# HKU-BAL/MegaPath-Nano

Hardware: AMD Instinct MI355X
Metric: Gbp/min ONT reads aligned+species-assigned vs RefSeq, 1/2/4/8 MI355X (higher is better)
Workload: dtype int32

## Files before the change

megapath_nano_amd/csrc/align.hip:

```cpp
#include "map_types.h"
#include "ext_kernels.h"
#include "fin_kernels.h"
#include "tag_kernels.h"
#include "stitch_kernels.h"
#include "plan_kernels.h"
#include "hit_kernels.h"
#include "mapper_internal.h"
#include "../../include/mpn_map.h"
#include "../../include/mpn_ssw.h"

#include <algorithm>
#include <condition_variable>
#include <deque>
#include <math.h>
#include <stdio.h>
#include <string.h>
#include <thread>
#include <pthread.h>
#include <time.h>
#include <atomic>
#include <functional>
#include <mutex>
#include <stdlib.h>
#include <string>
// ... 764 lines not shown
    int n_jobs = 0;
};

struct HostSeqs { const char *seqs; const int64_t *seq_off; const int32_t *seq_len; const int64_t *tseq_off; };

static int run_job_group(const RefView &rv, const mpn_map_opt *opt, int nj_cap, const unsigned long long *d_nj, DevRound &dv, const uint8_t *d_reads,
                         const int64_t *d_read_off, const int32_t *d_read_len, int64_t budget, const HostSeqs *hs, StreamLease &st) {
    if (nj_cap == 0) return 0;
    int nj = nj_cap;
    WallTimer wt;
    Slot &SL = *tl_slot;
    const int strip_scores = ext_strip_scores_ok(opt->a, -opt->b, -opt->sc_ambi, opt->q + opt->e, opt->q2 + opt->e2) ? 1 : 0;
    ExtParams prm;
    prm.sc_mch = (int8_t)opt->a; prm.sc_mis = (int8_t)-opt->b; prm.sc_n = (int8_t)-opt->sc_ambi;
    prm.q = (int8_t)opt->q; prm.e = (int8_t)opt->e; prm.q2 = (int8_t)opt->q2; prm.e2 = (int8_t)opt->e2; prm.zdrop_thres = opt->zdrop;
    prm.zdrop_inv = opt->zdrop_inv; prm.max_gap = opt->max_gap;
    const size_t order_cap = (size_t)nj + (size_t)N_STRIP * 8 + 16;
    if (SL.pool_sizes.ensure((size_t)nj * sizeof(JobSizes) + 16) || SL.pool_buckets.ensure((size_t)2 * N_BUCKETS * 4 + sizeof(LayoutTotals) + 16) ||
        SL.pool_order.ensure(order_cap * 4) || SL.pin_res.ensure(sizeof(LayoutTotals) + 96) ||
        SL.pool_redo_ids.ensure((size_t)nj * 4 + 16) || SL.pool_probes.ensure((size_t)nj * sizeof(InvProbe) + 16))
        return -1;
    struct { ExtJob *p; } d_jobs{dv.jobs};
    JobSizes *d_sizes = SL.pool_sizes.as<JobSizes>();
    int32_t *d_bcnt = SL.pool_buckets.as<int32_t>(), *d_bcur = d_bcnt + N_BUCKETS;
    LayoutTotals *d_tot = reinterpret_cast<LayoutTotals *>(d_bcnt + 2 * N_BUCKETS);
    struct { int32_t *p; } d_order{SL.pool_order.as<int32_t>()};
    {
        ZeroList z{};
        zero_list_push(z, d_bcnt, (size_t)2 * N_BUCKETS * 4 + sizeof(LayoutTotals));
        zero_list_push(z, dv.used + 1, 8);
        zero_list_push(z, dv.used + 5, 8);
        zero_list_push(z, dv.used + 8, 16);
        zero_list_push(z, dv.used + 7, 8);
        MPN_HIP_CHECK(zero_regions(z, st));
    }
    const int lay_grid = std::max(1, std::min((nj + 255) / 256, 256));
    EvTimer evl(st);
    static const bool tiled_on = []() { const char *e = getenv("MPN_TILED"); return !e || atoi(e) != 0; }();
    static const int tile_pick = []() { const char *e = getenv("MPN_TILE_CLASS"); return e ? std::min(std::max(atoi(e), 0), N_TILE_CLASS - 1) : -1; }();
    hipLaunchKernelGGL(job_classify_kernel, dim3(lay_grid), dim3(256), 0, st, d_jobs.p, d_nj, strip_scores, prm, g_force_kernel ? g_force_kernel : (tiled_on ? 0 : 7),
                       tile_pick, d_sizes, d_bcnt, d_tot);
    hipLaunchKernelGGL(job_scan_kernel, dim3(1), dim3(1024), 0, st, d_sizes, d_nj, (const int32_t *)d_bcnt, d_bcur, d_tot, d_order.p);
    hipLaunchKernelGGL(job_layout_kernel, dim3(lay_grid), dim3(256), 0, st, d_jobs.p, d_nj, (const JobSizes *)d_sizes, d_bcur, d_order.p);
    MPN_HIP_CHECK(hipGetLastError());
    LayoutTotals *h_tot = SL.pin_res.as<LayoutTotals>();
    evl.mark(56);
    MPN_HIP_CHECK(hipMemcpyAsync(h_tot, d_tot, sizeof(LayoutTotals), hipMemcpyDeviceToHost, st));
    MPN_HIP_CHECK(stream_sync(st));
    evl.resolve();
    const LayoutTotals T = *h_tot;
    nj = T.n_jobs;
    dv.n_jobs = nj;
    if (nj == 0) return 0;
    if (T.too_large) { set_error("DP window too large for LDS staging (%d x %d)", T.tl_q, T.tl_t); return -4; }
    if (!dv.compact) {
        if (SL.pool_compact.ensure((size_t)T.cig_tot * 4 * 2 + 16)) return -1;
        dv.compact = SL.pool_compact.as<uint32_t>();
        dv.cig_cap = T.cig_tot;
    }
    if (budget > 0 && T.p_tot > budget && nj > 1) return 1;
    const int *cnt = T.cnt, *base = T.base;
    g_stats[4] += nj; g_stats[5] += T.cells; g_stats[31] += T.strip_cells[0] + T.strip_cells[1] + T.strip_cells[2];
    for (int c = 0; c < 3; ++c) g_stats[41 + c] += T.strip_cells[c];
    g_stats[58] += T.xstrip_cells;
    for (int c = 0; c < N_TILE_CLASS; ++c) {
        g_stats[64] += cnt[L_TILE + c];
        g_stats[STAT_TILE_CLASS + c] += cnt[L_TILE + c];
    }
    if (getenv("MPN_DEBUG_JOBS")) {
        static const char *const fam[] = {"wg64", "wg", "strip", "band", "tile"};
        for (int l = 0; l < N_LISTS; ++l)
            if (cnt[l]) fprintf(stderr, "[jobs] %s list %-2d n=%d\n", fam[l < L_WG ? 0 : l < L_STRIP ? 1 : l < L_BAND ? 2 : l < L_TILE ? 3 : 4], l, cnt[l]);
    }
    if (const char *dump = getenv("MPN_DUMP_STRIPS")) {
        const int n_ord = base[L_BAND] - base[L_STRIP];
        std::vector<int32_t> ord(n_ord);
        std::vector<ExtJob> hj(nj);
        MPN_HIP_CHECK(hipMemcpy(ord.data(), d_order.p + base[L_STRIP], (size_t)n_ord * 4, hipMemcpyDeviceToHost));
        MPN_HIP_CHECK(hipMemcpy(hj.data(), d_jobs.p, (size_t)nj * sizeof(ExtJob), hipMemcpyDeviceToHost));
        static std::mutex mu;
        std::lock_guard<std::mutex> lk(mu);
        if (const char *all = getenv("MPN_DUMP_JOBS"))
            if (FILE *f = fopen(all, "ab")) {
                for (int j = 0; j < nj; ++j) {
                    const int32_t rec[6] = {hj[j].cls, hj[j].qlen, hj[j].tlen, hj[j].w, hj[j].flag, hj[j].n_col};
                    fwrite(rec, 4, 6, f);
                }
                fclose(f);
            }
        if (FILE *f = fopen(dump, "ab")) {
            for (int l = L_STRIP; l < L_BAND; ++l)
                for (int k = base[l]; k < base[l + 1]; ++k) {
                    const int jid = ord[k - base[L_STRIP]];
                    const int32_t rec[4] = {strip_glc_of_list(l), jid >= 0 ? hj[jid].qlen : 0, jid >= 0 ? hj[jid].tlen : 0, jid >= 0 ? hj[jid].strip_s : 0};
                    fwrite(rec, 4, 4, f);
                }
            fclose(f);
        }
    }
    if (SL.pool_P.ensure((size_t)T.p_tot + 16) || SL.pool_OFF.ensure((size_t)T.row_tot * 2 * 4 + 16) ||
        SL.pool_state.ensure((size_t)T.state_tot + 16) || SL.pool_CIG.ensure((size_t)T.cig_tot * 4 + 16))
        return -1;
    wt.stop_into(g_stats[27]);
    struct { uint8_t *p; } P{SL.pool_P.as<uint8_t>()};
    struct { int32_t *p; } OFF{SL.pool_OFF.as<int32_t>()};
    struct { int8_t *p; } gstate{SL.pool_state.as<int8_t>()};
    struct { uint32_t *p; } CIG{SL.pool_CIG.as<uint32_t>()};
    struct { ExtRes *p; } d_res{dv.res};
    uint32_t *d_compact = dv.compact;
    unsigned long long *d_used = dv.used;
    int32_t *d_redo_ids = SL.pool_redo_ids.as<int32_t>();
    InvProbe *d_probes = SL.pool_probes.as<InvProbe>();
    auto launch_list = [&](int l, const int32_t *ord, int n, hipStream_t s) -> int {
        if (n == 0) return 0;
        if (l < L_STRIP) {
            const int ntc = (l - L_LDS) / 5;
            const size_t lds = std::max<size_t>((size_t)T.lds_need[(l - L_LDS) % 5], 64);
#define MPN_WG_LAUNCH(NT)                                                                                                             \
            do {                                                                                                                      \
                if (lds > 64 * 1024) MPN_HIP_CHECK(hipFuncSetAttribute((const void *)ext_dp_wg_kernel<NT>, hipFuncAttributeMaxDynamicSharedMemorySize, (int)lds)); \
                hipLaunchKernelGGL(ext_dp_wg_kernel<NT>, dim3(n), dim3(NT), lds, s, d_jobs.p, ord, n, prm, d_reads, d_read_off, d_read_len, \
                                   rv, P.p, OFF.p, gstate.p, d_res.p);                                                                \
            } while (0)
            if (ntc == 0) MPN_WG_LAUNCH(64); else if (ntc == 1) MPN_WG_LAUNCH(256); else if (ntc == 2) MPN_WG_LAUNCH(512); else MPN_WG_LAUNCH(1024);
#undef MPN_WG_LAUNCH
        } else if (l < L_BAND) {
            const int fam = (l - L_STRIP) / 48;
            StripSegs segs;
            segs.n = 0;
            int blocks = 0;
            size_t lds = 0;
            const int c_lo = fam == 0 ? 0 : 3, c_hi = fam == 0 ? 3 : N_STRIP_CLASS;
            for (int glc = 2; glc >= 0; --glc)
                for (int sclass = c_lo + glc; sclass < c_hi; sclass += 3) {
                    const int l0 = L_STRIP + 16 * sclass, nl = base[l0 + 16] - base[l0], per = strip_windows_per_wave(l0);
                    if (nl == 0) continue;
                    const int stride = (std::max(T.strip_lds[sclass], 16) + 3) & ~3;
                    const int nr_stride = fam ? T.strip_nr[sclass] + 16 : 0;
                    lds = std::max(lds, (size_t)stride * per + STRIP_TAB_BYTES + (size_t)per * 8 * nr_stride);
                    segs.s[segs.n++] = StripSeg{blocks, nl, base[l0], stride, nr_stride, glc, sclass >= 6 ? 1 : 0};
                    blocks += nl / per;
                }
            if (blocks == 0) return 0;
#define MPN_STRIP_LAUNCH(EX)                                                                                                          \
            do {                                                                                                                      \
                if (lds > 64 * 1024) MPN_HIP_CHECK(hipFuncSetAttribute((const void *)ext_dp_strip_kernel<EX>, hipFuncAttributeMaxDynamicSharedMemorySize, (int)lds)); \
                hipLaunchKernelGGL(ext_dp_strip_kernel<EX>, dim3(blocks), dim3(64), lds, s, d_jobs.p, (const int32_t *)d_order.p, segs, prm, d_reads, \
                                   d_read_off, d_read_len, rv, P.p, d_res.p);                                                         \
            } while (0)
            if (fam == 0) MPN_STRIP_LAUNCH(false); else MPN_STRIP_LAUNCH(true);
#undef MPN_STRIP_LAUNCH
        } else if (l >= L_TILE) {
            const int c = l - L_TILE;
            const size_t lds = (size_t)std::max(T.tile_lds[c], 64);
#define MPN_TILE_LAUNCH(S, NW)                                                                                                        \
            do {                                                                                                                      \
                if (lds > 64 * 1024) MPN_HIP_CHECK(hipFuncSetAttribute((const void *)ext_dp_tile_kernel<S, NW>, hipFuncAttributeMaxDynamicSharedMemorySize, (int)lds)); \
                hipLaunchKernelGGL((ext_dp_tile_kernel<S, NW>), dim3(n), dim3(64 * NW), lds, s, d_jobs.p, ord, n, prm, d_reads, d_read_off, \
                                   d_read_len, rv, P.p, gstate.p, d_res.p, d_used + 7);                                              \
            } while (0)
            static_assert(N_TILE_CLASS == 4, "tile classes");
            if (c == 0) MPN_TILE_LAUNCH(16, 1); else if (c == 1) MPN_TILE_LAUNCH(4, 8); else if (c == 2) MPN_TILE_LAUNCH(8, 4); else MPN_TILE_LAUNCH(4, 16);
#undef MPN_TILE_LAUNCH
        } else {
            const int bvar = (l - L_BAND) / 4;
            const size_t lds = std::max<size_t>((size_t)T.band_lds[(l - L_BAND) % 4], 64);
// ... 2080 lines not shown
```

megapath_nano_amd/csrc/ext_kernels.h:

```cpp
#pragma once
#include "mpn_common.h"
#include "map_types.h"

namespace mpn {

enum { EZ_APPROX_MAX = 0x02, EZ_RIGHT = 0x08, EZ_EXTZ_ONLY = 0x40, EZ_REV_CIGAR = 0x80 };

struct ExtJob {
    int32_t read;
    int32_t rid;
    int32_t rev;
    int32_t qs, qlen;
    int32_t ts, tlen;
    int32_t reversed;
    int32_t w, zdrop, end_bonus, flag;
    int64_t p_off;
    int64_t row_off;
    int64_t cig_off;
    int32_t n_col;
    int32_t state_mode;
    int64_t state_off;
    int32_t layout;
    int32_t qstride;
    int32_t strip_s;
// ... 852 lines not shown
                                                         const int n_list, const ExtParams &prm, const uint8_t *__restrict__ reads,
                                                         const int64_t *__restrict__ read_off, const int32_t *__restrict__ read_len,
                                                         const RefView &rv, uint8_t *__restrict__ P, ExtRes *__restrict__ res, uint8_t *smem,
                                                         const int lds_stride, const int nr_stride) {
    const int j0 = first < n_list ? order[first] : -1;
    if (j0 < 0) return;
    const int S = jobs[j0].strip_s;
#define MPN_CASE(SS) case SS: ext_strip_exact<SS, GL, RIGHT>(jobs, order, first, n_list, prm, reads, read_off, read_len, rv, P, res, smem, lds_stride, nr_stride); break
    switch (S) {
        MPN_CASE(1); MPN_CASE(2); MPN_CASE(3); MPN_CASE(4); MPN_CASE(5); MPN_CASE(6); MPN_CASE(7); MPN_CASE(8);
        MPN_CASE(9); MPN_CASE(10); MPN_CASE(11); MPN_CASE(12); MPN_CASE(13); MPN_CASE(14); MPN_CASE(15);
        default: ext_strip_exact<16, GL, RIGHT>(jobs, order, first, n_list, prm, reads, read_off, read_len, rv, P, res, smem, lds_stride, nr_stride); break;
    }
#undef MPN_CASE
}

struct StripSeg { int32_t first_block, n_list, ord_off, lds_stride, nr_stride, glc, right; };
struct StripSegs { StripSeg s[6]; int32_t n; };

template <bool EXACT>
__global__ __launch_bounds__(64) __attribute__((amdgpu_waves_per_eu(3, 3))) void ext_dp_strip_kernel(const ExtJob *__restrict__ jobs, const int32_t *__restrict__ order, StripSegs segs,
                                                          ExtParams prm, const uint8_t *__restrict__ reads,
                                                          const int64_t *__restrict__ read_off, const int32_t *__restrict__ read_len,
                                                          RefView rv, uint8_t *__restrict__ P, ExtRes *__restrict__ res) {
    extern __shared__ __attribute__((aligned(16))) uint8_t smem[];
    int k = 0;
    while (k + 1 < segs.n && (int)blockIdx.x >= segs.s[k + 1].first_block) ++k;
    const StripSeg sg = segs.s[k];
    const int32_t *ord = order + sg.ord_off;
    if constexpr (!EXACT) {
        {
            const int first2 = ((int)blockIdx.x - sg.first_block) * (8 >> sg.glc);
            int S = 16;
            for (int k = 0; k < (8 >> sg.glc); ++k) { const int slot = first2 + k; if (slot < sg.n_list && ord[slot] >= 0) { S = jobs[ord[slot]].strip_s; break; } }
#define MPN_PAIR(SS, GLN) ext_strip_pair<SS, GLN>(jobs, ord, first2, sg.n_list, prm, reads, read_off, read_len, rv, P, res, smem, sg.lds_stride)
#define MPN_PAIR_S(GLN) switch (S) { case 1: MPN_PAIR(1, GLN); break; case 2: MPN_PAIR(2, GLN); break; case 3: MPN_PAIR(3, GLN); break; case 4: MPN_PAIR(4, GLN); break; \
            case 5: MPN_PAIR(5, GLN); break; case 6: MPN_PAIR(6, GLN); break; case 7: MPN_PAIR(7, GLN); break; case 8: MPN_PAIR(8, GLN); break; \
            case 9: MPN_PAIR(9, GLN); break; case 10: MPN_PAIR(10, GLN); break; case 11: MPN_PAIR(11, GLN); break; case 12: MPN_PAIR(12, GLN); break; \
            case 13: MPN_PAIR(13, GLN); break; case 14: MPN_PAIR(14, GLN); break; case 15: MPN_PAIR(15, GLN); break; default: MPN_PAIR(16, GLN); break; }
            if (sg.glc == 0) MPN_PAIR_S(16) else if (sg.glc == 1) MPN_PAIR_S(32) else MPN_PAIR_S(64)
#undef MPN_PAIR_S
#undef MPN_PAIR
        }
    } else {
        const int first = ((int)blockIdx.x - sg.first_block) * (4 >> sg.glc);
#define MPN_GL(GLN, RT) ext_strip_exact_dispatch<GLN, RT>(jobs, ord, first, sg.n_list, prm, reads, read_off, read_len, rv, P, res, smem, sg.lds_stride, sg.nr_stride)
        if (sg.right) { if (sg.glc == 0) MPN_GL(16, true); else if (sg.glc == 1) MPN_GL(32, true); else MPN_GL(64, true); }
        else { if (sg.glc == 0) MPN_GL(16, false); else if (sg.glc == 1) MPN_GL(32, false); else MPN_GL(64, false); }
#undef MPN_GL
    }
}

struct TileGeom { int T0, rows, n_lanes, W, jlo, jhi; int64_t base; };
__host__ __device__ inline TileGeom tile_geom(int tile, int qlen, int tlen, int w, int S) {
    const int R = 64 * S;
    TileGeom g{};
    g.T0 = tile * R;
    g.rows = tlen - g.T0 < R ? tlen - g.T0 : R;
    g.n_lanes = (g.rows + S - 1) / S;
    g.W = g.n_lanes * S;
    g.jlo = g.T0 - w > 0 ? g.T0 - w : 0;
    g.jhi = g.T0 + g.rows - 1 + w < qlen - 1 ? g.T0 + g.rows - 1 + w : qlen - 1;
    const int64_t m = tile;
    const int64_t k0 = (int64_t)w / R + 1;
    const int64_t n0 = m > k0 ? m - k0 : 0;
    const int64_t s_lo = (int64_t)R * (n0 * (k0 + m - 1) / 2) - n0 * (int64_t)w;
    const int64_t num = (int64_t)qlen - R - w;
    int64_t k1 = num <= 0 ? 0 : (num + R - 1) / R;
    if (k1 > m) k1 = m;
    const int64_t s_hi = (int64_t)R * (k1 * (k1 - 1) / 2) + k1 * (int64_t)(R - 1 + w) + (m - k1) * (int64_t)(qlen - 1);
    g.base = (s_hi - s_lo + 64 * m) * R;
    return g;
}
__host__ __device__ inline int64_t tile_matrix_bytes(int qlen, int tlen, int w, int S) {
    const int R = 64 * S, nt_all = (tlen + R - 1) / R, nt_band = (int)(((int64_t)qlen - 1 + w) / R) + 1, nt = nt_all < nt_band ? nt_all : nt_band;
    const TileGeom g = tile_geom(nt - 1, qlen, tlen, w, S);
    return g.base + (int64_t)((g.jhi >= g.jlo ? g.jhi - g.jlo + 1 : 0) + g.n_lanes - 1) * g.W;
}
__host__ __device__ inline bool ext_tile_ok(int qlen, int tlen, int w) {
    const int d = qlen > tlen ? qlen - tlen : tlen - qlen;
    return qlen > 0 && tlen > 0 && w >= 1 && d <= w && tlen <= 32768 && qlen <= 60000;
}

__host__ __device__ inline bool ext_tile_exact_ok(int mch, int mis, int amb, int q, int e, int q2, int e2, int qlen, int tlen, int w) {
    if (!(qlen > 0 && tlen > 0 && w >= 1 && tlen <= 8191 && qlen <= 16384 && qlen + tlen - 1 <= 14000)) return false;
    const int mn = qlen < tlen ? qlen : tlen, mx = qlen > tlen ? qlen : tlen;
    int worst = mis < amb ? -mis : -amb;
    if (worst < 0) worst = 0;
    const int g1 = worst * mn + q + e * (mx - mn + 1), g1b = q + e * (mx + 1), g2 = worst * mn + q2 + e2 * (mx - mn + 1), g2b = q2 + e2 * (mx + 1);
    const int lo1 = g1 > g1b ? g1 : g1b, lo2 = g2 > g2b ? g2 : g2b;
    return mch * mn < 32000 && (lo1 < lo2 ? lo1 : lo2) < 32000;
}
constexpr int TILE_RING_COLS = 2048, TILE_CTRL_BYTES = 4 * (2 * 16 + 4);
__host__ __device__ inline int ext_tile_ring_off(int qlen) { return ((qlen + 3) & ~3) + 64 + TILE_CTRL_BYTES; }
__host__ __device__ inline int ext_tile_lds_bytes(int qlen, int tlen, bool exact, int NW) {
    return ext_tile_ring_off(qlen) + (NW > 1 ? 12 * TILE_RING_COLS : 0) + (exact ? 8 * ((qlen + tlen + 2) & ~3) : 0);
}
__host__ __device__ inline bool ext_tile_pipe_ok(int w, int S, int NW) {
    return 2 * w + 128 < NW * (TILE_RING_COLS / NW + 64 * S);
}
constexpr int TILE_SPIN_MAX = 1 << 21;

template <int S, int NW, bool EXACT, bool RIGHT>
__device__ __forceinline__ void ext_tile_body(const ExtJob &jb, const int jid, const ExtParams &prm, const uint8_t *__restrict__ reads,
                                              const int64_t *__restrict__ read_off, const int32_t *__restrict__ read_len, const RefView &rv,
                                              uint8_t *__restrict__ P, int8_t *__restrict__ gstate, ExtRes *__restrict__ res, uint8_t *smem,
                                              unsigned long long *__restrict__ n_failed) {
    static_assert(S % 4 == 0 && S <= 16 && NW >= 1 && NW <= 16, "rows per lane: 4, 8, 12 or 16");
    constexpr int R = 64 * S, NT = 64 * NW;
    const int tid = threadIdx.x, lane = tid & 63, wave = tid >> 6;
    const int qlen = jb.qlen, tlen = jb.tlen;
    int q = prm.q, e = prm.e, q2 = prm.q2, e2 = prm.e2;
    if (q2 + e2 < q + e) { int t_ = q; q = q2; q2 = t_; t_ = e; e = e2; e2 = t_; }
    const int qe = q + e, qe2 = q2 + e2;
    int w = jb.w;
    if (w < 0) w = tlen > qlen ? tlen : qlen;
    ExtRes out;
    out.max = 0; out.zdropped = 0; out.max_q = out.max_t = out.mqe_t = -1; out.mqe = NEG_INF; out.score = NEG_INF;
    out.reach_end = 0; out.n_cigar = 0; out.r_done = -1; out.bt_i = out.bt_j = -1; out.do_bt = 0; out.zcode = 0; out.cig_pos = 0;
    if (!(EXACT ? ext_tile_exact_ok(prm.sc_mch, prm.sc_mis, prm.sc_n, prm.q, prm.e, prm.q2, prm.e2, qlen, tlen, w) : ext_tile_ok(qlen, tlen, w)) || -prm.sc_mis > 2 * (q + e) ||
        (NW > 1 && !ext_tile_pipe_ok(w, S, NW))) { if (tid == 0) res[jid] = out; return; }
    constexpr int RS = RIGHT ? 0 : 4, RA = RIGHT ? 1 : 3, RB = 2, RA2 = RIGHT ? 3 : 1, RB2 = RIGHT ? 4 : 0;
    const uint32_t sb_mch = (uint32_t)(8 * prm.sc_mch + RS + 128) & 0xff, sb_mis = (uint32_t)(8 * prm.sc_mis + RS + 128) & 0xff,
                   sb_n = (uint32_t)(8 * prm.sc_n + RS + 128) & 0xff;
    const int q_pad = (qlen + 3) & ~3;
    uint32_t *tab = reinterpret_cast<uint32_t *>(smem + q_pad);
    if (tid < 5) tab[tid] = lane == 4 ? sb_n * 0x01010101u : (sb_mis * 0x01010101u) ^ ((sb_mch ^ sb_mis) << (8 * lane));
    {
        const int64_t roff = read_off[jb.read];
        const int32_t rlen = read_len[jb.read];
        for (int i = tid; i < qlen; i += NT) smem[i] = (uint8_t)(4 * ext_qbase(reads, roff, rlen, jb.rev, jb.qs + (jb.reversed ? qlen - 1 - i : i)));
    }
    int long_thres = e != e2 ? (q2 - q) / (e - e2) - 1 : 0;
    if (q2 + e2 + long_thres * e2 > q + e + long_thres * e) ++long_thres;
    const int long_diff = long_thres * (e - e2) - (q2 - q) - e2;
#define MPN_BND(R) (8 * ((R) == 0 ? -qe : (R) < long_thres ? -e : (R) == long_thres ? long_diff : -e2))
    typedef short s16x2 __attribute__((ext_vector_type(2)));
    typedef unsigned short u16x2 __attribute__((ext_vector_type(2)));
    auto pk = [](int lo, int hi) { return (uint32_t)(hi * 65536 + lo); };
    constexpr int BETA = 0x2000 + 128;
    const int cv_lo = -8 * qe + RA + BETA, cv_hi = -8 * qe2 + RA2 + BETA, cu_lo = -8 * qe + RB + BETA, cu_hi = -8 * qe2 + RB2 + BETA;
    const uint32_t CV = pk(cv_lo, cv_hi), CU = pk(cu_lo, cu_hi);
    const uint32_t FRESH_U = pk(-8 * qe, -8 * qe) + CU, EDGE_V = pk(-8 * qe, -8 * qe) + CV;
    const uint32_t KONST = sb_n | 0x2000u;
    const uint32_t KZZ = pk(-16 * qe + RA + RB + BETA, -16 * qe2 + RA2 + RB2 + BETA);
    constexpr int RU = RIGHT ? 8 : 0;
    const uint32_t KEA = pk(8 * e - 8 * qe + RA - RU, 8 * e2 - 8 * qe2 + RA2 - RU), KEB = pk(8 * e - 8 * qe + RB - RU, 8 * e2 - 8 * qe2 + RB2 - RU);
    const uint32_t EIGHT = 0x00080008u, RANK_CLR = 0xfff8fff8u;
    const uint32_t MCH7 = (uint32_t)(8 * prm.sc_mch + 7 + BETA) * 0x00010001u;
    const int64_t g0 = rv.seq_off[jb.rid] + jb.ts;
    uint32_t *bnd_base = reinterpret_cast<uint32_t *>(gstate + jb.state_off);
    const int n_tiles = (tlen + R - 1) / R;
    uint32_t *ctrl = reinterpret_cast<uint32_t *>(smem + ext_tile_ring_off(qlen) - TILE_CTRL_BYTES);
    uint32_t *ring = ctrl + TILE_CTRL_BYTES / 4;
    constexpr int C = TILE_RING_COLS / NW;
    const int n_r = qlen + tlen - 1;
    uint32_t *BEST = reinterpret_cast<uint32_t *>(smem + ext_tile_ring_off(qlen) + (NW > 1 ? 12 * TILE_RING_COLS : 0)), *SE = BEST + ((n_r + 3) & ~3);
    int32_t *HL = reinterpret_cast<int32_t *>(NW > 1 ? bnd_base : bnd_base + 6 * (size_t)qlen);
    if (tid < 2 * NW + 1) ctrl[tid] = 0;
    if constexpr (EXACT) {
        for (int r = tid; r < n_r; r += NT) {
            int st = 0, en = tlen - 1;
            if (st < r - qlen + 1) st = r - qlen + 1;
            if (en > r) en = r;
            if (st < (r - w + 1) >> 1) st = (r - w + 1) >> 1;
            if (en > (r + w) >> 1) en = (r + w) >> 1;
            if (st > en) { st = 1; en = 0; }
            BEST[r] = 0;
            SE[r] = (uint32_t)st | (uint32_t)en << 16;
        }
        for (int t = tid; t < tlen; t += NT) HL[t] = NEG_INF;
        __builtin_amdgcn_fence(__ATOMIC_RELEASE, "agent");
    }
    __syncthreads();
    const bool head = lane == 0;
    int32_t score8 = 0;
    uint32_t *const prod_in = &ctrl[(wave + NW - 1) % NW], *const cons_in = &ctrl[NW + (wave + NW - 1) % NW];
    uint32_t *const prod_out = &ctrl[wave], *const cons_out = &ctrl[NW + wave];
    uint32_t *const ring_in = ring + 3 * C * ((wave + NW - 1) % NW), *const ring_out = ring + 3 * C * wave;
    uint32_t n_in = 0, n_out = 0, seen_prod = 0, seen_cons = 0;
    bool failed = false;
    auto wait_gt = [&](uint32_t *ctr, uint32_t lim, uint32_t &seen) -> bool {
        if ((int)(seen - lim) > 0) return true;
        for (int k = 0; k < TILE_SPIN_MAX; ++k) {
            seen = __hip_atomic_load(ctr, __ATOMIC_RELAXED, __HIP_MEMORY_SCOPE_WORKGROUP);
            if ((int)(seen - lim) > 0) return true;
            if (__hip_atomic_load(&ctrl[2 * NW], __ATOMIC_RELAXED, __HIP_MEMORY_SCOPE_WORKGROUP)) return false;
            __builtin_amdgcn_s_sleep(1);
        }
        __hip_atomic_store(&ctrl[2 * NW], 1u, __ATOMIC_RELAXED, __HIP_MEMORY_SCOPE_WORKGROUP);
        return false;
    };
    for (int tile = NW > 1 ? wave : 0; tile < n_tiles; tile += NW) {
        const TileGeom G = tile_geom(tile, qlen, tlen, w, S);
        const int T0 = G.T0, n_lanes = G.n_lanes, W = G.W, jlo = G.jlo, jhi = G.jhi;
        if (jhi < jlo) break;
        const int prev_jhi = tile > 0 ? min(qlen - 1, T0 - 1 + w) : -1;
        const int jlo_next = T0 + R - w > 0 ? T0 + R - w : 0;
        uint32_t *bnd_in = bnd_base + (size_t)(tile & 1) * 3 * (size_t)qlen, *bnd_out = bnd_base + (size_t)((tile + 1) & 1) * 3 * (size_t)qlen;
        const bool write_bnd = tile + 1 < n_tiles;
        const int t0 = T0 + lane * S;
        uint32_t UL[S], YL[S], TSEL[S];
        int32_t H8[S];
#pragma unroll
        for (int k = 0; k < S; ++k) {
            const int t = t0 + k;
            const int sq = t < tlen ? ref_code(rv, g0 + (jb.reversed ? tlen - 1 - t : t)) : 4;
            TSEL[k] = 0x0c0c0100u | (sq < 4 ? 4u + (uint32_t)sq : 0u);
            UL[k] = jlo == 0 ? pk(MPN_BND(t), MPN_BND(t)) + CU : FRESH_U;
            YL[k] = 0;
            H8[k] = 8 * (t < long_thres ? -(q + e * (t + 1)) : -(q2 + e2 * (t + 1)));
        }
        uint8_t *prow = P + jb.p_off + G.base + (int64_t)lane * S;
        const int n_steps = (jhi - jlo + 1) + n_lanes - 1;
        int out_v = 0, out_x = 0, out_h = 0;
        uint32_t qt = 0;
        auto qcode = [&](int col) -> uint32_t { return col < qlen ? (uint32_t)smem[col] : 16u; };
        uint32_t qt_next = *reinterpret_cast<const uint32_t *>(reinterpret_cast<const uint8_t *>(tab) + qcode(jlo));
        uint32_t qc_next = qcode(jlo + 1);
        uint32_t bv_n = 0, bx_n = 0, bh_n = 0, bv_n2 = 0, bx_n2 = 0, bh_n2 = 0;
        auto load_bnd = [&](int col, uint32_t &a, uint32_t &b, uint32_t &c) {
            if (tile > 0 && head && col <= prev_jhi && col < qlen) {
                if constexpr (NW == 1) { a = bnd_in[3 * (size_t)col]; b = bnd_in[3 * (size_t)col + 1]; c = bnd_in[3 * (size_t)col + 2]; }
                else {
                    const uint32_t n = n_in + (uint32_t)(col - jlo), slot = n % C;
                    if (!failed && !wait_gt(prod_in, n, seen_prod)) failed = true;
                    __atomic_signal_fence(__ATOMIC_SEQ_CST);
                    a = ring_in[slot]; b = ring_in[C + slot]; c = ring_in[2 * C + slot];
                    __atomic_signal_fence(__ATOMIC_SEQ_CST);
                    __hip_atomic_store(cons_in, n + 1, __ATOMIC_RELAXED, __HIP_MEMORY_SCOPE_WORKGROUP);
                }
            }
        };
        load_bnd(jlo, bv_n, bx_n, bh_n);
        load_bnd(jlo + 1, bv_n2, bx_n2, bh_n2);
        for (int step = 0; step < n_steps; ++step) {
            const uint32_t q_in = qt_next;
            qt_next = *reinterpret_cast<const uint32_t *>(reinterpret_cast<const uint8_t *>(tab) + qc_next);
            qc_next = qcode(jlo + step + 2);
            const uint32_t bv = bv_n, bx = bx_n, bh = bh_n;
            bv_n = bv_n2; bx_n = bx_n2; bh_n = bh_n2;
            load_bnd(jlo + step + 2, bv_n2, bx_n2, bh_n2);
            const uint32_t qt_s = (uint32_t)wave_shr1_zero((int)qt);
            const int v_s = wave_shr1_zero(out_v), x_s = wave_shr1_zero(out_x), h_s = wave_shr1_zero(out_h);
            const int j = jlo + step - lane;
            qt = head ? q_in : qt_s;
            uint32_t Vp, Xp;
            int32_t Hup;
            if (head) {
                if (tile == 0) { const int bj = MPN_BND(j); Vp = pk(bj, bj) + CV; Xp = 0; Hup = 0; }
                else { Vp = bv; Xp = bx; Hup = (int32_t)bh; }
            } else { Vp = (uint32_t)v_s; Xp = (uint32_t)x_s; Hup = h_s; }
            if (j >= jlo && j <= jhi && lane < n_lanes) {
                uint32_t dw[S / 4], ecell[4] = {0, 0, 0, 0};
                const int d_in = j - t0 + w;
                const int d_out = j - t0 - w;
#pragma unroll
                for (int k = 0; k < S; ++k) {
                    const bool enter = d_in == k, edge = d_out == k;
                    const uint32_t Up = enter ? FRESH_U : UL[k];
                    const uint32_t Yl = enter ? 0u : YL[k];
                    Vp = edge ? EDGE_V : Vp;
                    Xp = edge ? 0u : Xp;
                    const uint32_t sc16 = __builtin_amdgcn_perm(qt, KONST, TSEL[k]);
                    const uint32_t A = Xp + Vp, B = Yl + Up;
                    const uint32_t M = __builtin_bit_cast(uint32_t, __builtin_elementwise_max(__builtin_bit_cast(s16x2, A), __builtin_bit_cast(s16x2, B)));
                    uint32_t m2, z16;
                    asm("v_pk_max_i16 %0, %1, %1 op_sel:[0,1] op_sel_hi:[1,0]" : "=v"(m2) : "v"(M));
                    asm("v_max_i16 %0, %1, %2" : "=v"(z16) : "v"(m2), "v"(sc16));
                    uint32_t zc;
                    asm("v_pk_min_i16 %0, %1, %2 op_sel_hi:[0,1]" : "=v"(zc) : "v"(z16), "v"(MCH7));
                    const uint32_t Zc = zc & RANK_CLR;
                    const uint32_t ZZ = Zc + KZZ;
                    const uint32_t nu = ZZ - Vp, nv = ZZ - Up;
                    u16x2 An = __builtin_elementwise_sub_sat(__builtin_bit_cast(u16x2, A), __builtin_bit_cast(u16x2, Zc + KEA));
                    u16x2 Bn = __builtin_elementwise_sub_sat(__builtin_bit_cast(u16x2, B), __builtin_bit_cast(u16x2, Zc + KEB));
                    uint32_t HA, HB;
                    asm("v_pk_min_u16 %0, %1, %2" : "=v"(HA) : "v"(__builtin_bit_cast(uint32_t, An)), "v"(EIGHT));
                    asm("v_pk_min_u16 %0, %1, %2" : "=v"(HB) : "v"(__builtin_bit_cast(uint32_t, Bn)), "v"(EIGHT));
                    if constexpr (RIGHT) {
                        An = __builtin_elementwise_sub_sat(An, __builtin_bit_cast(u16x2, EIGHT));
                        Bn = __builtin_elementwise_sub_sat(Bn, __builtin_bit_cast(u16x2, EIGHT));
                    }
                    uint32_t Fw;
                    asm("v_lshl_or_b32 %0, %1, 1, %2" : "=v"(Fw) : "v"(HB), "v"(HA));
                    asm("v_and_or_b32 %0, %1, 7, %2" : "=v"(ecell[k & 3]) : "v"(z16), "v"(Fw));
                    const int32_t h_left = H8[k] + (int32_t)(nv & 0xffffu) - cv_lo, h_up = Hup + (int32_t)(nu & 0xffffu) - cu_lo;
                    const int32_t h = enter ? h_up : h_left;
                    H8[k] = h;
                    Hup = h;
                    if constexpr (EXACT) {
                        const int t = t0 + k, r = t + j;
                        const uint32_t se = SE[r < n_r ? r : n_r - 1];
                        const int st_ = (int)(se & 0xffffu), en_ = (int)(se >> 16);
                        const bool inb = t >= st_ && t <= en_;
                        const int en1 = st_ + ((en_ - st_) & ~3);
                        const int cls = t == en_ ? 0 : t < en1 ? 1 + ((t - st_) & 3) : 5;
                        const uint32_t word = (uint32_t)((h >> 3) + 32768) << 16 | (0xffffu - ((uint32_t)cls << 13 | (uint32_t)t));
                        atomicMax(&BEST[r < n_r ? r : n_r - 1], inb ? word : 0u);
                        if (inb && j == qlen - 1) HL[t] = h >> 3;
                    }
                    UL[k] = nu; YL[k] = __builtin_bit_cast(uint32_t, Bn);
                    Vp = nv; Xp = __builtin_bit_cast(uint32_t, An);
                    if ((k & 3) == 3) {
                        uint32_t e01, e23;
                        asm("v_lshl_or_b32 %0, %1, 8, %2" : "=v"(e01) : "v"(ecell[1]), "v"(ecell[0]));
                        asm("v_lshl_or_b32 %0, %1, 8, %2" : "=v"(e23) : "v"(ecell[3]), "v"(ecell[2]));
                        const uint32_t lo = __builtin_amdgcn_perm(e23, e01, 0x05040100u), hi = __builtin_amdgcn_perm(e23, e01, 0x07060302u);
                        asm("v_lshl_or_b32 %0, %1, 2, %2" : "=v"(dw[k >> 2]) : "v"(hi), "v"(lo));
                    }
                }
                out_v = (int)Vp; out_x = (int)Xp; out_h = Hup;
                if constexpr (S == 16) *reinterpret_cast<uint4 *>(prow + (int64_t)step * W) = make_uint4(dw[0], dw[1], dw[2], dw[3]);
                else if constexpr (S == 8) *reinterpret_cast<uint2 *>(prow + (int64_t)step * W) = make_uint2(dw[0], dw[1]);
                else if constexpr (S == 4) *reinterpret_cast<uint32_t *>(prow + (int64_t)step * W) = dw[0];
                if constexpr (NW == 1) {
                    if (write_bnd && lane == 63) { bnd_out[3 * (size_t)j] = (uint32_t)out_v; bnd_out[3 * (size_t)j + 1] = (uint32_t)out_x; bnd_out[3 * (size_t)j + 2] = (uint32_t)out_h; }
                } else if (write_bnd && lane == 63 && j >= jlo_next) {
                    const uint32_t n = n_out + (uint32_t)(j - jlo_next), slot = n % C;
                    if (!failed && !wait_gt(cons_out, n - C, seen_cons)) failed = true;
                    __atomic_signal_fence(__ATOMIC_SEQ_CST);
                    ring_out[slot] = (uint32_t)out_v; ring_out[C + slot] = (uint32_t)out_x; ring_out[2 * C + slot] = (uint32_t)out_h;
                    __atomic_signal_fence(__ATOMIC_SEQ_CST);
                    __hip_atomic_store(prod_out, n + 1, __ATOMIC_RELAXED, __HIP_MEMORY_SCOPE_WORKGROUP);
                }
            }
        }
        if (tile + 1 == n_tiles) {
            const int lt = tlen - 1 - T0, ll = lt / S, kk = lt % S;
            int32_t hv = 0;
#pragma unroll
            for (int k = 0; k < S; ++k) hv = k == kk ? H8[k] : hv;
            score8 = __shfl(hv, ll);
        }
        if constexpr (NW == 1) {
            __builtin_amdgcn_fence(__ATOMIC_RELEASE, "agent");
            __syncthreads();
            __builtin_amdgcn_fence(__ATOMIC_ACQUIRE, "agent");
        } else {
            if (tile > 0 && prev_jhi >= jlo) n_in += (uint32_t)(prev_jhi - jlo + 1);
            if (write_bnd && jhi >= jlo_next) n_out += (uint32_t)(jhi - jlo_next + 1);
        }
    }
#undef MPN_BND
    if constexpr (NW > 1) {
        __builtin_amdgcn_fence(__ATOMIC_RELEASE, "agent");
        __syncthreads();
        __builtin_amdgcn_fence(__ATOMIC_ACQUIRE, "agent");
        if (wave != (EXACT ? 0 : (n_tiles - 1) % NW)) return;
        if (__hip_atomic_load(&ctrl[2 * NW], __ATOMIC_RELAXED, __HIP_MEMORY_SCOPE_WORKGROUP)) {
            if (lane == 0) { res[jid] = out; atomicAdd(n_failed, 1ull); }
            return;
        }
    }
    if constexpr (!EXACT) {
        if (lane == 0) {
            out.score = score8 >> 3;
            out.r_done = qlen + tlen - 2;
            out.do_bt = 1; out.bt_i = tlen - 1; out.bt_j = qlen - 1;
            res[jid] = out;
        }
    } else {
        if constexpr (NW == 1) __syncthreads();
        const int tlm1 = tlen - 1;
        struct Best { int m, t, r; };
        auto scan_first_max = [&](Best x) {
#pragma unroll
            for (int d = 1; d < 64; d <<= 1) {
                const Best o{__shfl_up(x.m, d), __shfl_up(x.t, d), __shfl_up(x.r, d)};
                if (lane >= d && !(x.m > o.m)) x = o;
            }
            return x;
        };
        auto diag = [&](int r, int &H, int &mt) {
            const uint32_t pv = BEST[r];
            H = pv ? (int)(pv >> 16) - 32768 : NEG_INF;
            mt = (int)((0xffffu - (pv & 0xffffu)) & 8191u);
        };
        int r_lim = n_r;
        for (int r = lane; r < n_r; r += 64) { const uint32_t se = SE[r]; if ((int)(se & 0xffffu) > (int)(se >> 16)) { r_lim = r; break; } }
        r_lim = wave_reduce_min(r_lim);
        const int n_eff = r_lim < n_r ? r_lim : n_r;
        const int C = (n_eff + 63) / 64, rlo = min(n_eff, lane * C), rhi = min(n_eff, rlo + C);
        auto chunk_best = [&](int lim) {
            Best b{NEG_INF, -1, -1};
            for (int r = rlo; r < rhi && r <= lim; ++r) { int H, mt; diag(r, H, mt); if (H > b.m) b = Best{H, mt, r}; }
            return b;
        };
        Best incl = scan_first_max(chunk_best(n_eff));
        Best in{__shfl_up(incl.m, 1), __shfl_up(incl.t, 1), __shfl_up(incl.r, 1)};
        ExtApply ez; ez.max = 0; ez.max_t = ez.max_q = -1; ez.zdropped = 0;
        if (lane > 0 && in.m > 0) { ez.max = in.m; ez.max_t = in.t; ez.max_q = in.r - in.t; }
        int r_break = n_eff;
        for (int r = rlo; r < rhi; ++r) {
            int H, mt; diag(r, H, mt);
            if (ext_apply_zdrop(ez, H, r, mt, jb.zdrop, e2)) { r_break = r; break; }
        }
        r_break = wave_reduce_min(r_break);
        const bool zd = r_break < n_eff;
        const bool dropped = zd || n_eff < n_r;
        const int r_last = zd ? r_break : n_eff - 1;
        Best fin = scan_first_max(chunk_best(r_last));
        fin = Best{__shfl(fin.m, 63), __shfl(fin.t, 63), __shfl(fin.r, 63)};
        __builtin_amdgcn_fence(__ATOMIC_ACQUIRE, "agent");
        const int t_lim = min(tlm1, r_last - (qlen - 1));
        const int Ct = (tlen + 63) / 64, tlo = min(tlen, lane * Ct), thi = min(tlen, tlo + Ct);
        Best me{NEG_INF, -1, -1};
        for (int t = tlo; t < thi && t <= t_lim; ++t) { const int h = HL[t]; if (h > me.m) me = Best{h, t, t}; }
        me = scan_first_max(me);
        me = Best{__shfl(me.m, 63), __shfl(me.t, 63), 0};
        if (lane == 0) {
            if (fin.m > 0) { out.max = fin.m; out.max_t = fin.t; out.max_q = fin.r - fin.t; }
            out.zdropped = dropped ? 1 : 0;
            if (me.m > NEG_INF) { out.mqe = me.m; out.mqe_t = me.t; }
            if (!dropped) out.score = HL[tlm1];
            out.r_done = dropped ? (zd ? r_break : n_eff) : n_r - 1;
            if (!dropped && !(jb.flag & EZ_EXTZ_ONLY)) { out.do_bt = 1; out.bt_i = tlen - 1; out.bt_j = qlen - 1; }
            else if (!dropped && (jb.flag & EZ_EXTZ_ONLY) && out.mqe + jb.end_bonus > out.max) { out.reach_end = 1; out.do_bt = 1; out.bt_i = out.mqe_t; out.bt_j = qlen - 1; }
            else if (out.max_t >= 0 && out.max_q >= 0) { out.do_bt = 1; out.bt_i = out.max_t; out.bt_j = out.max_q; }
            res[jid] = out;
        }
    }
}

template <int S, int NW>
__global__ __launch_bounds__(64 * NW) void ext_dp_tile_kernel(const ExtJob *__restrict__ jobs, const int32_t *__restrict__ order, int n_jobs,
                                                              ExtParams prm, const uint8_t *__restrict__ reads,
                                                              const int64_t *__restrict__ read_off, const int32_t *__restrict__ read_len,
                                                              RefView rv, uint8_t *__restrict__ P, int8_t *__restrict__ gstate, ExtRes *__restrict__ res,
                                                              unsigned long long *__restrict__ n_failed) {
    extern __shared__ __attribute__((aligned(16))) uint8_t smem[];
    const int jid = order[blockIdx.x];
    const ExtJob jb = jobs[jid];
#define MPN_TB(EX, RT) ext_tile_body<S, NW, EX, RT>(jb, jid, prm, reads, read_off, read_len, rv, P, gstate, res, smem, n_failed)
    if (jb.flag & EZ_APPROX_MAX) MPN_TB(false, false);
    else if (jb.flag & EZ_RIGHT) MPN_TB(true, true);
    else MPN_TB(true, false);
#undef MPN_TB
}



__device__ __forceinline__ void ext_bt_band(int rr, int qlen, int tlen, int bw, int &st, int &en) {
    st = 0; en = tlen - 1;
    if (st < rr - qlen + 1) st = rr - qlen + 1;
    if (en > rr) en = rr;
    if (st < (rr - bw + 1) >> 1) st = (rr - bw + 1) >> 1;
    if (en > (rr + bw) >> 1) en = (rr + bw) >> 1;
}
__device__ __forceinline__ int ext_bt_force(int i, int st, int en) {
    int force_state = -1;
    if (i < st) force_state = 2;
    if (i > en) force_state = 1;
    return force_state;
}
__device__ __forceinline__ int ext_bt_decode(int b, bool rank_is_op) { return rank_is_op ? b : (b & ~7) | (4 - (b & 7)); }
__device__ __forceinline__ int ext_bt_next_state(int state, int tmp, int force_state) {
    if (state == 0) state = tmp & 7;
    else if (!(tmp >> (state + 2) & 1)) state = 0;
    if (state == 0) state = tmp & 7;
    if (force_state >= 0) state = force_state;
    return state;
}

__global__ __launch_bounds__(64) void ext_bt_kernel(const ExtJob *__restrict__ jobs, const int32_t *__restrict__ order, int n_jobs,
                                                    const uint8_t *__restrict__ P, const int32_t *__restrict__ OFF,
                                                    uint32_t *__restrict__ CIG, uint32_t *__restrict__ COMPACT,
                                                    unsigned long long *__restrict__ compact_used, ExtRes *__restrict__ res) {
    const int k = blockIdx.x * blockDim.x + threadIdx.x;
    const int jid = k < n_jobs ? order[k] : -1;
    const bool live = jid >= 0;
    ExtJob jb = jobs[live ? jid : 0];
    ExtRes r = res[live ? jid : 0];
    const bool walk = live && r.do_bt;
    if (live && !r.do_bt) res[jid].cig_pos = 0;
    if (!walk) { jb.qlen = jb.tlen = 1; r.bt_i = r.bt_j = -1; }
    const int n_col = jb.n_col, n_r = jb.qlen + jb.tlen - 1;
    const uint8_t *p = P + jb.p_off;
    const int32_t *off = OFF + 2 * jb.row_off, *off_end = off + n_r;
    const bool rowmajor = jb.layout == 1;
    const bool rank_is_op = (jb.flag & EZ_RIGHT) != 0;
    const bool byslot = jb.layout == 2;
    const bool tiled = jb.layout == 3;
    TileGeom tg{};
    int tg_tile = -1;
    const int bw = jb.w < 0 ? (jb.tlen > jb.qlen ? jb.tlen : jb.qlen) : jb.w;
    const bool rev_cigar = (jb.flag & EZ_REV_CIGAR) != 0;
    uint32_t *cend = CIG + jb.cig_off;
    const int cap = jb.qlen + jb.tlen + 2;
    uint32_t *cbeg = cend - cap;
    int n = 0, i = r.bt_i, j = r.bt_j, state = 0;
    uint32_t cur_op = 0xf, cur_len = 0;
#define MPN_FLUSH() do { if (cur_len) { if (rev_cigar) cbeg[n] = cur_len << 4 | cur_op; else cend[-1 - n] = cur_len << 4 | cur_op; ++n; } } while (0)
#define MPN_PUSHOP(OP, LEN) do { if ((uint32_t)(OP) == cur_op) cur_len += (LEN); else { MPN_FLUSH(); cur_op = (OP); cur_len = (LEN); } } while (0)
    constexpr int BT_AHEAD = 8;
    while (i >= 0 && j >= 0) {
        const int rr = i + j;
        int force_state = -1, tmp;
        if (rowmajor) {
            if (state == 0) {
                uint8_t ahead[BT_AHEAD];
#pragma unroll
                for (int k = 0; k < BT_AHEAD; ++k) {
                    const int ii = i - k, jj = j - k;
                    ahead[k] = (ii >= 0 && jj >= 0) ? p[(int64_t)(jj + ii / jb.strip_s) * jb.qstride + ii] : (uint8_t)0xff;
                }
                int k = 0;
                tmp = 0;
#pragma unroll
                for (int q = 0; q < BT_AHEAD; ++q) {
                    if (k != q) continue;
                    if (i - q < 0 || j - q < 0) continue;
                    const int b = ext_bt_decode(ahead[q], rank_is_op);
                    if ((b & 7) == 0) ++k; else tmp = b;
                }
                if (k > 0) { MPN_PUSHOP(0, (uint32_t)k); i -= k; j -= k; }
                if (k == BT_AHEAD || i < 0 || j < 0) continue;
            } else {
                tmp = ext_bt_decode(p[(int64_t)(j + i / jb.strip_s) * jb.qstride + i], rank_is_op);
            }
        }
        else if (tiled) {
            int st, en;
            ext_bt_band(rr, jb.qlen, jb.tlen, bw, st, en);
            force_state = ext_bt_force(i, st, en);
            tmp = 0;
            if (force_state < 0) {
                const int tile = i / (64 * jb.strip_s);
                if (tile != tg_tile) { tg = tile_geom(tile, jb.qlen, jb.tlen, bw, jb.strip_s); tg_tile = tile; }
                const int lt = i - tg.T0;
                tmp = ext_bt_decode(p[tg.base + (int64_t)((j - tg.jlo) + lt / jb.strip_s) * tg.W + lt], rank_is_op);
            }
// ... 392 lines not shown
```

Before: 14.93.

## Accumulate per-antidiagonal best in registers and cut per-cell LDS atomics

In the exact tile DP path, each lane now keeps per-cell running maxima of the packed score/position word in registers, with band start/length slots that shift along the anti-diagonals. It issues one LDS atomicMax per step (plus a flush at the last row) instead of an atomic and an SE lookup for every cell. It also adds an edge correction (qe) for the last-column score on a specific anti-diagonal and writes a header record to the job dump. The aim is to remove LDS atomic contention and repeated band decoding from the inner loop, at the cost of more registers and subtle correctness risk in the shifted band bookkeeping and score packing.

```diff
diff --git a/megapath_nano_amd/csrc/align.hip b/megapath_nano_amd/csrc/align.hip
--- a/megapath_nano_amd/csrc/align.hip
+++ b/megapath_nano_amd/csrc/align.hip
@@ -870,6 +870,8 @@
         std::lock_guard<std::mutex> lk(mu);
         if (const char *all = getenv("MPN_DUMP_JOBS"))
             if (FILE *f = fopen(all, "ab")) {
+                const int32_t head[6] = {-2, nj, 0, 0, 0, 0};
+                fwrite(head, 4, 6, f);
                 for (int j = 0; j < nj; ++j) {
                     const int32_t rec[6] = {hj[j].cls, hj[j].qlen, hj[j].tlen, hj[j].w, hj[j].flag, hj[j].n_col};
                     fwrite(rec, 4, 6, f);
diff --git a/megapath_nano_amd/csrc/ext_kernels.h b/megapath_nano_amd/csrc/ext_kernels.h
--- a/megapath_nano_amd/csrc/ext_kernels.h
+++ b/megapath_nano_amd/csrc/ext_kernels.h
@@ -958,6 +958,14 @@
     return qlen > 0 && tlen > 0 && w >= 1 && d <= w && tlen <= 32768 && qlen <= 60000;
 }
 
+__device__ __forceinline__ void ext_bt_band(int rr, int qlen, int tlen, int bw, int &st, int &en) {
+    st = 0; en = tlen - 1;
+    if (st < rr - qlen + 1) st = rr - qlen + 1;
+    if (en > rr) en = rr;
+    if (st < (rr - bw + 1) >> 1) st = (rr - bw + 1) >> 1;
+    if (en > (rr + bw) >> 1) en = (rr + bw) >> 1;
+}
+
 __host__ __device__ inline bool ext_tile_exact_ok(int mch, int mis, int amb, int q, int e, int q2, int e2, int qlen, int tlen, int w) {
     if (!(qlen > 0 && tlen > 0 && w >= 1 && tlen <= 8191 && qlen <= 16384 && qlen + tlen - 1 <= 14000)) return false;
     const int mn = qlen < tlen ? qlen : tlen, mx = qlen > tlen ? qlen : tlen;
@@ -1036,11 +1044,8 @@
     if (tid < 2 * NW + 1) ctrl[tid] = 0;
     if constexpr (EXACT) {
         for (int r = tid; r < n_r; r += NT) {
-            int st = 0, en = tlen - 1;
-            if (st < r - qlen + 1) st = r - qlen + 1;
-            if (en > r) en = r;
-            if (st < (r - w + 1) >> 1) st = (r - w + 1) >> 1;
-            if (en > (r + w) >> 1) en = (r + w) >> 1;
+            int st, en;
+            ext_bt_band(r, qlen, tlen, w, st, en);
             if (st > en) { st = 1; en = 0; }
             BEST[r] = 0;
             SE[r] = (uint32_t)st | (uint32_t)en << 16;
@@ -1086,6 +1091,19 @@
             UL[k] = jlo == 0 ? pk(MPN_BND(t), MPN_BND(t)) + CU : FRESH_U;
             YL[k] = 0;
             H8[k] = 8 * (t < long_thres ? -(q + e * (t + 1)) : -(q2 + e2 * (t + 1)));
+        }
+        uint32_t ACC[S], se_in = 0;
+        int ST[S], LEN[S];
+        auto se_at = [&](int r) -> uint32_t { return SE[r < n_r ? r : n_r - 1]; };
+        auto band_slot = [](uint32_t se, int &st, int &len) {
+            st = (int)(se & 0xffffu); len = (int)(se >> 16) - st;
+            if (len < 0) { st = 0x4000; len = 0; }
+        };
+        auto in_band = [](int d, int len) { return (uint32_t)d <= (uint32_t)len; };
+        if constexpr (EXACT) {
+#pragma unroll
+            for (int k = 0; k < S; ++k) { ACC[k] = 0; band_slot(se_at(t0 + jlo + k), ST[k], LEN[k]); }
+            se_in = se_at(t0 + jlo + S);
         }
         uint8_t *prow = P + jb.p_off + G.base + (int64_t)lane * S;
         const int n_steps = (jhi - jlo + 1) + n_lanes - 1;
@@ -1131,6 +1149,8 @@
                 uint32_t dw[S / 4], ecell[4] = {0, 0, 0, 0};
                 const int d_in = j - t0 + w;
                 const int d_out = j - t0 - w;
+                uint32_t se_new = 0;
+                if constexpr (EXACT) { se_new = se_in; se_in = se_at(t0 + j + S + 1); }
 #pragma unroll
                 for (int k = 0; k < S; ++k) {
                     const bool enter = d_in == k, edge = d_out == k;
@@ -1166,15 +1186,11 @@
                     H8[k] = h;
                     Hup = h;
                     if constexpr (EXACT) {
-                        const int t = t0 + k, r = t + j;
-                        const uint32_t se = SE[r < n_r ? r : n_r - 1];
-                        const int st_ = (int)(se & 0xffffu), en_ = (int)(se >> 16);
-                        const bool inb = t >= st_ && t <= en_;
-                        const int en1 = st_ + ((en_ - st_) & ~3);
-                        const int cls = t == en_ ? 0 : t < en1 ? 1 + ((t - st_) & 3) : 5;
-                        const uint32_t word = (uint32_t)((h >> 3) + 32768) << 16 | (0xffffu - ((uint32_t)cls << 13 | (uint32_t)t));
-                        atomicMax(&BEST[r < n_r ? r : n_r - 1], inb ? word : 0u);
-                        if (inb && j == qlen - 1) HL[t] = h >> 3;
+                        const int t = t0 + k, d = t - ST[k], len = LEN[k];
+                        const bool inb = in_band(d, len);
+                        const int cls = d == len ? 0 : d < (len & ~3) ? 1 + (d & 3) : 5;
+                        const uint32_t word = ((((uint32_t)h << 13) + 0x80000000u) & 0xffff0000u) | (0xffffu - ((uint32_t)cls << 13 | (uint32_t)t));
+                        ACC[k] = max(ACC[k], inb ? word : 0u);
                     }
                     UL[k] = nu; YL[k] = __builtin_bit_cast(uint32_t, Bn);
                     Vp = nv; Xp = __builtin_bit_cast(uint32_t, An);
@@ -1187,6 +1203,24 @@
                     }
                 }
                 out_v = (int)Vp; out_x = (int)Xp; out_h = Hup;
+                if constexpr (EXACT) {
+                    const int r0 = t0 + j;
+                    atomicMax(&BEST[r0], ACC[0]);
+                    if (j == qlen - 1) {
+#pragma unroll
+                        for (int k = 0; k < S; ++k)
+                            if (in_band(t0 + k - ST[k], LEN[k])) HL[t0 + k] = H8[k] >> 3;
+                    }
+                    if (j == jhi) {
+#pragma unroll
+                        for (int k = 1; k < S; ++k)
+                            if (r0 + k < n_r) atomicMax(&BEST[r0 + k], ACC[k]);
+                    }
+#pragma unroll
+                    for (int k = 0; k + 1 < S; ++k) { ACC[k] = ACC[k + 1]; ST[k] = ST[k + 1]; LEN[k] = LEN[k + 1]; }
+                    ACC[S - 1] = 0;
+                    band_slot(se_new, ST[S - 1], LEN[S - 1]);
+                }
                 if constexpr (S == 16) *reinterpret_cast<uint4 *>(prow + (int64_t)step * W) = make_uint4(dw[0], dw[1], dw[2], dw[3]);
                 else if constexpr (S == 8) *reinterpret_cast<uint2 *>(prow + (int64_t)step * W) = make_uint2(dw[0], dw[1]);
                 else if constexpr (S == 4) *reinterpret_cast<uint32_t *>(prow + (int64_t)step * W) = dw[0];
@@ -1248,9 +1282,11 @@
             }
             return x;
         };
+        const int r_edge = tlen >= 2 && 2 * tlm1 + w < n_r ? 2 * tlm1 + w : -1;
+        auto last_col_h = [&](int t) { const int h = HL[t]; return h > NEG_INF && t == tlm1 && r_edge == n_r - 1 ? h + qe : h; };
         auto diag = [&](int r, int &H, int &mt) {
             const uint32_t pv = BEST[r];
-            H = pv ? (int)(pv >> 16) - 32768 : NEG_INF;
+            H = pv ? (int)(pv >> 16) - 32768 + (r == r_edge ? qe : 0) : NEG_INF;
             mt = (int)((0xffffu - (pv & 0xffffu)) & 8191u);
         };
         int r_lim = n_r;
@@ -1282,14 +1318,14 @@
         const int t_lim = min(tlm1, r_last - (qlen - 1));
         const int Ct = (tlen + 63) / 64, tlo = min(tlen, lane * Ct), thi = min(tlen, tlo + Ct);
         Best me{NEG_INF, -1, -1};
-        for (int t = tlo; t < thi && t <= t_lim; ++t) { const int h = HL[t]; if (h > me.m) me = Best{h, t, t}; }
+        for (int t = tlo; t < thi && t <= t_lim; ++t) { const int h = last_col_h(t); if (h > me.m) me = Best{h, t, t}; }
         me = scan_first_max(me);
         me = Best{__shfl(me.m, 63), __shfl(me.t, 63), 0};
         if (lane == 0) {
             if (fin.m > 0) { out.max = fin.m; out.max_t = fin.t; out.max_q = fin.r - fin.t; }
             out.zdropped = dropped ? 1 : 0;
             if (me.m > NEG_INF) { out.mqe = me.m; out.mqe_t = me.t; }
-            if (!dropped) out.score = HL[tlm1];
+            if (!dropped) out.score = last_col_h(tlm1);
             out.r_done = dropped ? (zd ? r_break : n_eff) : n_r - 1;
             if (!dropped && !(jb.flag & EZ_EXTZ_ONLY)) { out.do_bt = 1; out.bt_i = tlen - 1; out.bt_j = qlen - 1; }
             else if (!dropped && (jb.flag & EZ_EXTZ_ONLY) && out.mqe + jb.end_bonus > out.max) { out.reach_end = 1; out.do_bt = 1; out.bt_i = out.mqe_t; out.bt_j = qlen - 1; }
@@ -1317,13 +1353,6 @@
 
 
 
-__device__ __forceinline__ void ext_bt_band(int rr, int qlen, int tlen, int bw, int &st, int &en) {
-    st = 0; en = tlen - 1;
-    if (st < rr - qlen + 1) st = rr - qlen + 1;
-    if (en > rr) en = rr;
-    if (st < (rr - bw + 1) >> 1) st = (rr - bw + 1) >> 1;
-    if (en > (rr + bw) >> 1) en = (rr + bw) >> 1;
-}
 __device__ __forceinline__ int ext_bt_force(int i, int st, int en) {
     int force_state = -1;
     if (i < st) force_state = 2;
```

New measurement: 15.09 (median of 6 runs). 1.01x the previous value.
